# TalShor/SciLMM

Measured on AMD Instinct MI355X. Metric: REML factorize+solve nnz(L)/s (simulated pedigree, fp64), higher is better.
Workload: dtype f64

## Files before the change

### scilmm_amd/csrc/dev.h

```cpp
#pragma once
#include <hip/hip_runtime.h>

#include <algorithm>
#include <cstdlib>
#include <optional>
#include <string>
#include <type_traits>
#include <vector>

#include "../../include/scilmm_hip.h"
#include "plan_types.h"
#include "handles.h"

namespace scilmm {

struct Tuning {
  int reserve_cus = 0;
  int side_streams = 2;
  bool no_mfma = false;
  bool trsm_lite = true;
  std::optional<bool> dense;
  std::optional<bool> outside;
  bool outside_merge = true;
  std::optional<int> outside_chunks;
  bool outside_prio = false;
  std::optional<double> cell_limit;
  bool no_lookahead = false;
  int look_depth = 2;
  bool host_cells = false;
  bool no_splitk = false;
  int64_t target_items = 1024;
  int64_t min_item = 24;
  int64_t max_item = 96;
  std::optional<int64_t> dense_items;
  int64_t dense_fill = 256;
  std::optional<bool> dense_taper;
  std::optional<int> dist_group;
  bool dist_nosplit = false;
  int chain_cap = 2048;
  int chain_wide = 12;
  bool no_chain = false;
  int64_t push_slice = 512;
  bool shadow = true;
  int chain_wide_t = 256;
  int chain_full_t = 768;
  bool sinv_generic = false;
};

inline Tuning read_tuning() {
  Tuning t;
  const char* gate = getenv("SCILMM_TUNING");
  if (!(gate && gate[0] == '1')) return t;
  auto env = [](const char* name) { return getenv(name); };
  auto is1 = [&](const char* name) { const char* e = env(name); return e && e[0] == '1'; };
  auto not0 = [&](const char* name) { const char* e = env(name); return !(e && e[0] == '0'); };
  const char* e;
  if ((e = env("SCILMM_RESERVE_CUS"))) t.reserve_cus = atoi(e);
  if ((e = env("SCILMM_SIDE_STREAMS"))) t.side_streams = atoi(e);
  t.no_mfma = is1("SCILMM_NO_MFMA");
  t.trsm_lite = not0("SCILMM_TRSM_LITE");
  if ((e = env("SCILMM_DENSE"))) t.dense = e[0] != '0';
  if ((e = env("SCILMM_OUTSIDE"))) t.outside = e[0] != '0';
  t.outside_merge = not0("SCILMM_OUTSIDE_MERGE");
  if ((e = env("SCILMM_OUTSIDE_CHUNKS"))) t.outside_chunks = atoi(e);
  t.outside_prio = is1("SCILMM_OUTSIDE_PRIO");
  if ((e = env("SCILMM_CELL_LIMIT"))) t.cell_limit = atof(e);
  t.no_lookahead = is1("SCILMM_NO_LOOKAHEAD");
  if ((e = env("SCILMM_LOOK_DEPTH"))) t.look_depth = std::max(1, atoi(e));
  t.host_cells = is1("SCILMM_HOST_CELLS");
  t.no_splitk = is1("SCILMM_NO_SPLITK");
  if ((e = env("SCILMM_TARGET_ITEMS"))) t.target_items = atoll(e);
  if ((e = env("SCILMM_MIN_ITEM"))) t.min_item = atoll(e);
  if ((e = env("SCILMM_MAX_ITEM"))) t.max_item = atoll(e);
  if ((e = env("SCILMM_DENSE_ITEMS"))) t.dense_items = atoll(e);
  if ((e = env("SCILMM_DENSE_FILL"))) t.dense_fill = atoll(e);
  if ((e = env("SCILMM_DENSE_TAPER"))) t.dense_taper = e[0] == '1';
  if ((e = env("SCILMM_DIST_GROUP"))) t.dist_group = atoi(e);
  t.dist_nosplit = is1("SCILMM_DIST_NOSPLIT");
  if ((e = env("SCILMM_CHAIN_CAP"))) t.chain_cap = atoi(e);
  if ((e = env("SCILMM_CHAIN_WIDE"))) t.chain_wide = atoi(e);
  t.no_chain = is1("SCILMM_NO_CHAIN");
  if ((e = env("SCILMM_PUSH_SLICE"))) t.push_slice = atoll(e);
  t.shadow = not0("SCILMM_SHADOW");
  if ((e = env("SCILMM_CHAIN_WIDE_T"))) t.chain_wide_t = atoi(e);
  if ((e = env("SCILMM_CHAIN_FULL_T"))) t.chain_full_t = atoi(e);
  t.sinv_generic = is1("SCILMM_SINV_GENERIC");
  return t;
}

inline bool verbose() { return getenv("SCILMM_VERBOSE") != nullptr; }

struct Dev {
  int device = 0;
  hipStream_t stream = nullptr;
  Tuning tune;
  int prio_lo = 0, prio_hi = 0;
  DevSym v{};
  std::vector<void*> allocs;
  int32_t* d_level_tiles = nullptr;
  int32_t* d_level_fronts = nullptr;
  int32_t* d_level_pairs = nullptr;
  int32_t* d_all_fronts = nullptr;
  std::vector<double*> vals;
  std::vector<uint8_t> have_vals;
  double* W = nullptr;
  double* X = nullptr;
  double* IO = nullptr;
  size_t io_cap = 0;
  double* partial = nullptr;
  size_t partial_cap = 0;
  double* d_out = nullptr;
  bool use_mfma = true;
  bool trsm_lite = true;
  hipEvent_t ev[8];
  scilmm_timing timing{};
  bool quad_pending = false;
  bool attrs_set = false;
  ComboDesc* d_combos = nullptr;
  UpdWork* d_work = nullptr;
  std::vector<int64_t> work_ptr;
  UpdWork* d_work_early = nullptr;
  std::vector<int64_t> early_ptr;
  int64_t max_slots = 0;
  hipStream_t side = nullptr;
  hipStream_t side2 = nullptr;
  hipStream_t side3 = nullptr;
  int nside = 2;
  bool serial_early = false;
  std::vector<hipEvent_t> lev_ev;
  hipEvent_t ev_asm = nullptr;
  hipEvent_t ev_x0 = nullptr, ev_x1 = nullptr;
  int32_t* d_tile_pslot = nullptr;
  int32_t* d_tile_pnseg = nullptr;
  int32_t* d_tile_pslot_e = nullptr;
  int32_t* d_tile_pnseg_e = nullptr;
  int32_t* d_red_tiles_e = nullptr;
  std::vector<int64_t> red_ptr_e;
  std::vector<int64_t> lev_cost_e, lev_cost_l;
// ... 23 lines not shown
  std::vector<int32_t> lv_ptr, lv_fronts, lv_tiles, lv_pairs;
  std::vector<int64_t> lv_tile_ptr, lv_tile_mid, lv_pair_ptr;
  int32_t* d_lmul_tiles = nullptr;
  int64_t n_lmul_tiles = 0;
  DenseWork* d_dwork_b = nullptr;
  std::vector<int64_t> dbatch_ptr;
  std::vector<hipEvent_t> batch_ev;
  std::vector<hipEvent_t> bpev;
  std::vector<int32_t> last_own_level;
  hipStream_t bstream = nullptr;
  hipStream_t comm = nullptr;
  std::vector<hipEvent_t> done_ev;
  double* ACC = nullptr;
  int32_t* d_col_front = nullptr;
  int64_t* d_yoff = nullptr;
  double* d_ybuf = nullptr;
  int32_t* d_sinv_pre_tiles = nullptr;
  std::vector<int64_t> sinv_pre_ptr;
  std::vector<int32_t> sinv_tail_front;
  int32_t* d_sinv_tail_fronts = nullptr;
  SinvWork* d_sinv_work = nullptr;
  std::vector<int64_t> sinv_work_ptr;
  bool work_external = false;
  bool outside_on = false;
  int32_t tail_level = 0;
  std::vector<uint8_t> outside_desc;
  OutsideWork* d_owork = nullptr;
  int32_t* d_grp_next = nullptr;
  int32_t* d_grp_t0 = nullptr;
  int64_t n_owork = 0;
  int32_t* d_tail_front = nullptr;
  uint8_t* d_keep_front = nullptr;
  hipStream_t outside_st = nullptr;
  std::vector<int64_t> ochunk_ptr;
  std::vector<hipEvent_t> out_evs;
  std::vector<int32_t> out_wait_chunk;
  bool dense_on = false;
  int front_bits = 64;
  double* d_zeros = nullptr;
  DenseWork* d_dwork_e = nullptr;
  DenseWork* d_dwork_l = nullptr;
  std::vector<int64_t> dwork_e_ptr, dwork_l_ptr;
  std::vector<int64_t> dwork_l_mid;
  int64_t n_late_split = 0;
  int look_depth = 2;
  int rhs_pending = -1;
  int32_t chain_T = 0, chain_l0 = 0;
  int32_t* d_chain = nullptr;
  int32_t* d_colmap = nullptr;
  int32_t* d_cf_ptr = nullptr;
  ChainPair* d_cf = nullptr;
  int32_t* d_cb_ptr = nullptr;
  ChainPair* d_cb = nullptr;
  int64_t* d_cg_ptr = nullptr;
  int32_t* d_cg_pairs = nullptr;
  int64_t chain_groups = 0;
  int32_t* d_cg_slot = nullptr;
  int32_t* d_fold = nullptr;
  int64_t n_fold = 0;
  double* d_push_partial = nullptr;
  int32_t* d_chain_flags = nullptr;
  int32_t* d_chain_err = nullptr;
  int32_t* h_chain_err = nullptr;
  int32_t chain_epoch = 0;
  std::vector<hipEvent_t> pev;
  bool det = false;
  PullPlan pull{};
  int32_t* d_pull_level_segs = nullptr;
  int32_t* d_pull_fold = nullptr;
  double* d_pull_partial = nullptr;
  uint8_t* d_chain_mask = nullptr;
  const int64_t* d_pat_rowptr = nullptr;
  const int64_t* d_pat_rowslot = nullptr;
  const int32_t* d_pat_rowcol = nullptr;
  int64_t n_float_atomic = 0;
  double* scan_partial = nullptr;
  size_t scan_partial_cap = 0;
  double* gram_partial = nullptr;
  size_t gram_partial_cap = 0;
  const int32_t* d_iperm = nullptr;
  hipEvent_t scan_ev[4] = {nullptr, nullptr, nullptr, nullptr};
  bool scan_pending = false;
  double scan_ms[3] = {0.0, 0.0, 0.0};
  hipEvent_t gxe_ev[2] = {nullptr, nullptr};
  bool gxe_pending = false;
  double gxe_ms[2] = {0.0, 0.0};
};

#define HIPCHK(call)                                                                                   \
  do {                                                                                                 \
    hipError_t _e = (call);                                                                            \
    if (_e != hipSuccess) {                                                                            \
      sym->err = std::string(#call) + ": " + hipGetErrorString(_e);                                    \
      return SCILMM_ERR_DEVICE;                                                                        \
    }                                                                                                  \
  } while (0)

#define TRY(call)                      \
  do {                                 \
    int _rc = (call);                  \
    if (_rc != SCILMM_OK) return _rc;  \
  } while (0)

struct DevScratch {
  std::string* const err;
  std::vector<void*> held;
// ... 100 lines not shown
```

### scilmm_amd/csrc/kernels.hip.h

```cpp
#pragma once
#include <hip/hip_runtime.h>
#ifndef SCILMM_UPD_WAVES
#define SCILMM_UPD_WAVES 2
#endif
#include <stdint.h>

#include "plan_types.h"

namespace scilmm {

typedef double d4 __attribute__((ext_vector_type(4)));

constexpr int NJB = NB / 16;
constexpr int KCS = 16;
constexpr int LDA = TM + 16;
constexpr int LDB = NB + 16;
constexpr int LDP = 34;

__device__ __forceinline__ d4 mfma_f64(double a, double b, d4 c) {
  return __builtin_amdgcn_mfma_f64_16x16x4f64(a, b, c, 0, 0, 0);
}

__global__ void k_assemble(int64_t nnz, const int64_t* __restrict__ dst, ValPtrs vp, double* __restrict__ L) {
  int64_t stride = (int64_t)gridDim.x * blockDim.x;
  for (int64_t e = (int64_t)blockIdx.x * blockDim.x + threadIdx.x; e < nnz; e += stride) {
    double v = 0.0;
#pragma unroll
    for (int k = 0; k < 8; ++k)
      if (k < vp.count) v += vp.s2[k] * vp.v[k][e];
    const int64_t d = dst[e];
    if (d >= 0) L[d] = v;
  }
}

__global__ void k_add_rows(int64_t count, const double* __restrict__ src, double* __restrict__ dst) {
  const int64_t i = (int64_t)blockIdx.x * blockDim.x + threadIdx.x;
  if (i < count) dst[i] += src[i];
}

__global__ void k_status_pack(const int32_t* __restrict__ status, double* __restrict__ out) { *out = (double)*status; }
__global__ void k_status_unpack(const double* __restrict__ in, int32_t* __restrict__ status) { *status = (int32_t)*in; }

__global__ void k_add_diag(int32_t n, const int64_t* __restrict__ diag_dst, ValPtrs vp, double* __restrict__ L) {
  int32_t j = blockIdx.x * blockDim.x + threadIdx.x;
  if (j >= n) return;
  double v = 0.0;
#pragma unroll
  for (int k = 0; k < 8; ++k)
    if (k < vp.count) v += vp.s2[k] * vp.v[k][j];
  if (diag_dst[j] >= 0) L[diag_dst[j]] += v;
}

template <bool MFMA>
__device__ __forceinline__ void tile_mma(const double* __restrict__ As, const double* __restrict__ Bs, int kc4, int ncb,
                                         int lane, int wv, d4 (&acc)[NJB][2]) {
  const int li = lane & 15, lk = lane >> 4;
  if (MFMA) {
    const double* ap = As + lk * LDA + 32 * wv + li;
// ... 1785 lines not shown
}

template <int MODE>
__global__ __launch_bounds__(256) void k_pull_fold(DevSym S, const int32_t* __restrict__ fold, const double* __restrict__ partial,
                                                   double* __restrict__ W, int32_t rp) {
  const int32_t s = fold[3 * blockIdx.x], slot0 = fold[3 * blockIdx.x + 1], ns = fold[3 * blockIdx.x + 2];
  const int c_lo = blockIdx.y * CW;
  const int rpl = min(CW, rp - c_lo);
  const int32_t c0 = S.sn_start[s], w = S.sn_start[s + 1] - c0;
  const int cc = threadIdx.x % CW;
  if (cc >= rpl) return;
  for (int k = threadIdx.x / CW; k < w; k += 256 / CW) {
    double sum = 0.0;
    for (int sl = 0; sl < ns; ++sl) sum += partial[((int64_t)(slot0 + sl) * NB + k) * rp + c_lo + cc];
    if (MODE == 0) W[(int64_t)(c0 + k) * rp + c_lo + cc] -= sum;
    else W[(int64_t)(c0 + k) * rp + c_lo + cc] = sum;
  }
}


__device__ __forceinline__ bool chain_wait(const int32_t* flag, int32_t epoch, int32_t* err, int behind) {
  int spins = 0;
  int32_t seen = __hip_atomic_load(err + 1, __ATOMIC_RELAXED, __HIP_MEMORY_SCOPE_AGENT);
  unsigned long long t_seen = wall_clock64();
  while (__hip_atomic_load(flag, __ATOMIC_RELAXED, __HIP_MEMORY_SCOPE_AGENT) < epoch) {
    if (behind == 0) __builtin_amdgcn_s_sleep(1);
    else
      for (int z = 0; z < min(behind, 8); ++z) __builtin_amdgcn_s_sleep(127);
    if ((++spins & 255) == 0) {
      if (__hip_atomic_load(err, __ATOMIC_RELAXED, __HIP_MEMORY_SCOPE_AGENT) != 0) return false;
      const int32_t now = __hip_atomic_load(err + 1, __ATOMIC_RELAXED, __HIP_MEMORY_SCOPE_AGENT);
      const unsigned long long t = wall_clock64();
      if (now != seen) {
        seen = now;
        t_seen = t;
      } else if (t - t_seen > 100000000ull) {
        __hip_atomic_store(err, 1, __ATOMIC_RELAXED, __HIP_MEMORY_SCOPE_AGENT);
        return false;
      }
    }
  }
  return true;
}

#ifndef SCILMM_CHAIN_WAVES
#define SCILMM_CHAIN_WAVES 2
#endif
#ifdef SCILMM_CHAIN_PROF
__device__ unsigned long long g_chain_prof[8 * 4096];
#define CPROF(slot) do { if (c == 0 && tid == 0 && i < 4096 && !BWD) g_chain_prof[8 * i + (slot)] = wall_clock64(); } while (0)
#else
#define CPROF(slot) do {} while (0)
#endif
template <bool MFMA, bool BWD, int NCTW>
__global__ __launch_bounds__(512, NCTW == 2 ? SCILMM_CHAIN_WAVES : 1) void k_chain(DevSym S, int32_t T, const int32_t* __restrict__ chain,
                                               const int32_t* __restrict__ pair_ptr, const ChainPair* __restrict__ pairs,
                                               const int32_t* __restrict__ colmap, const double* __restrict__ L,
                                               const double* __restrict__ invD, const double* W, double* X, int32_t rp,
                                               int32_t ncw, int32_t* flags, int32_t epoch, int32_t* err, int32_t* ticket) {
  constexpr int CW = 16 * NCTW, LDW = NCTW == 2 ? 48 : NCTW == 4 ? 80 : 112, NCT = NCTW;
  static_assert(NCTW == 2 || NCTW == 4 || NCTW == 7, "k_chain: 32-, 64- or 112-column windows");
  __shared__ __attribute__((aligned(16))) double Ys[NB * LDW];
  __shared__ int s_ok, s_ready, s_ticket;
  const int tid = threadIdx.x, lane = tid & 63, wv = tid >> 6;
  const int li = lane & 15, lk = lane >> 4;
  if (tid == 0) s_ticket = atomicAdd(ticket, 1);
  __syncthreads();
  const int32_t lin = s_ticket;
  const int32_t ord = lin / ncw, c = lin - ord * ncw;
  const int32_t i = BWD ? T - 1 - ord : ord;
  const int c_lo = c * CW;
  const int rpl = min(CW, rp - c_lo);
  const int ncn = rpl >> 4;
  const int32_t s = chain[i];
  const int32_t c0 = S.sn_start[s], w = S.sn_start[s + 1] - c0;
  const int32_t m = (int32_t)(S.sn_rowptr[s + 1] - S.sn_rowptr[s]);
  const double* I = invD + S.inv_off[s];
  constexpr int NK = NB / 4;
  const int jrow = 16 * wv + li;
  const int32_t e0 = pair_ptr[i], e1 = pair_ptr[i + 1];
  if (wv == 0) {
    int ready = 0;
    bool open = true;
    for (int32_t base = e0; base < e1 && open; base += 64) {
      bool r = false;
      if (base + lane < e1)
        r = __hip_atomic_load(flags + (int64_t)pairs[base + lane].other * ncw + c, __ATOMIC_RELAXED, __HIP_MEMORY_SCOPE_AGENT) >= epoch;
      const unsigned long long b = __ballot(r);
      const int lead = (~b == 0ull) ? 64 : __builtin_ctzll(~b);
      ready += lead;
      open = lead == 64;
    }
    if (lane == 0) s_ready = ready;
  }
  const int w4 = (w + 3) & ~3;
  const int kbeg = BWD ? 16 * wv : 0;
  const int kend = BWD ? w4 : min(w4, 16 * (wv + 1));
  double iv[NK];
  auto load_iv = [&]() {
    const int jc = jrow < w ? jrow : 0;
    const uint32_t voff = (uint32_t)(BWD ? jc * w + lk : lk * w + jc);
    const int klast = uniform_int(max(w4 - 4, 0)), wu = uniform_int(w);
    const double* Ib = invD + uniform_i64(S.inv_off[s]);
#pragma unroll
    for (int u = 0; u < NK; ++u) {
      const int ku = min(4 * u, klast);
      iv[u] = ld_off(Ib + (BWD ? ku : ku * wu), voff * 8u);
    }
  };
  const double* Yin = BWD ? (const double*)X : W;
  double yv[NCT][4];
  auto load_yv = [&]() {
#pragma unroll
    for (int cn = 0; cn < NCT; ++cn)
#pragma unroll
      for (int r = 0; r < 4; ++r) {
        const int jr = 16 * wv + lk + 4 * r;
        yv[cn][r] = (jr < w && cn < ncn) ? Yin[(int64_t)(c0 + jr) * rp + c_lo + 16 * cn + li] : 0.0;
      }
  };
  if (NCTW == 2) load_yv();
  d4 acc[NCT];
#pragma unroll
  for (int cn = 0; cn < NCT; ++cn) acc[cn] = (d4){0.0, 0.0, 0.0, 0.0};
  __syncthreads();
  const int32_t nready = s_ready;
  bool ok = true;
  auto load_frag = [&](int32_t e, double (&av)[NK]) {
    const ChainPair pr = pairs[e];
    if (!BWD) {
      const int32_t so = chain[pr.other];
      const int32_t wo = S.sn_start[so + 1] - S.sn_start[so];
      const int64_t md = S.sn_rowptr[so + 1] - S.sn_rowptr[so];
      int q = jrow - pr.jp0;
      if (pr.jp0 < 0) q = colmap[pr.map + jrow];
      const bool rowok = q >= 0 && q < pr.nq;
      const double* Pj = L + uniform_i64(S.sn_loff[so] + pr.p0);
      const int64_t mdu = uniform_int((int)md);
      const uint32_t voff = (uint32_t)(lk * (int)md + (rowok ? q : 0));
      const int klast = uniform_int(max(((wo + 3) & ~3) - 4, 0));
#pragma unroll
      for (int u = 0; u < NK; ++u) av[u] = ld_off(Pj + (int64_t)min(4 * u, klast) * mdu, voff * 8u);
    } else {
      const double* Pi = L + uniform_i64(S.sn_loff[s] + pr.p0);
      const uint32_t voff = (uint32_t)((jrow < w ? jrow : 0) * m + lk);
      const int klast = uniform_int(max(((pr.nq + 3) & ~3) - 4, 0));
#pragma unroll
      for (int u = 0; u < NK; ++u) av[u] = ld_off(Pi + min(4 * u, klast), voff * 8u);
    }
  };
  auto consume = [&](int32_t e, double (&av)[NK]) {
    const ChainPair pr = pairs[e];
    const int32_t so = chain[pr.other];
    const int32_t co = S.sn_start[so], wo = S.sn_start[so + 1] - co;
    const int kn = BWD ? ((pr.nq + 3) & ~3) : ((wo + 3) & ~3);
    bool rowok;
    if (!BWD) {
      int q = jrow - pr.jp0;
      if (pr.jp0 < 0) q = colmap[pr.map + jrow];
      rowok = q >= 0 && q < pr.nq;
    } else {
      rowok = jrow < w;
    }
    const int kvalid = BWD ? pr.nq : wo;
    if (NCTW == 2 && e == e1 - 1) load_iv();
    if (e - e0 >= nready) {
      if (tid == 0) s_ok = chain_wait(flags + (int64_t)pr.other * ncw + c, epoch, err, e1 - 1 - e) ? 1 : 0;
      if (e == e1 - 1) CPROF(0);
      __syncthreads();
      ok = s_ok != 0;
    }
    if (ok) {
      const int nx = BWD ? pr.nq : wo;
#pragma unroll
      for (int cbase = 0; cbase < LDW; cbase += 64) {
        const int cc = cbase + (tid & 63);
        if (cc < LDW) {
          double xv[NB / 8];
#pragma unroll
// ... 1 lines not shown
            const int k = (tid >> 6) + 8 * u;
            xv[u] = 0.0;
            if (k < nx && cc < rpl) {
              int64_t xr;
              if (!BWD) xr = co + k;
              else xr = (pr.jp0 >= 0) ? co + pr.jp0 + k : S.sn_rows[S.sn_rowptr[s] + pr.p0 + k];
              xv[u] = X[xr * rp + c_lo + cc];
            }
          }
#pragma unroll
          for (int u = 0; u < NB / 8; ++u) {
            const int k = (tid >> 6) + 8 * u;
            if (k < kn) Ys[k * LDW + cc] = xv[u];
          }
        }
      }
    }
    __syncthreads();
    if (e == e1 - 1) CPROF(1);
    if (ok) {
      if (MFMA) {
#pragma unroll
        for (int u = 0; u < NK; ++u)
          if (4 * u < kn) {
#pragma unroll
            for (int cn = 0; cn < NCT; ++cn)
              if (cn < ncn)
                acc[cn] = mfma_f64((rowok && 4 * u + lk < kvalid) ? av[u] : 0.0, Ys[(4 * u + lk) * LDW + 16 * cn + li], acc[cn]);
          }
      } else {
        for (int k = 0; k < kn; ++k) {
#pragma unroll
          for (int r = 0; r < 4; ++r) {
            const int jr = 16 * wv + lk + 4 * r;
            double a = 0.0;
            if (!BWD) {
              const int64_t md = S.sn_rowptr[so + 1] - S.sn_rowptr[so];
              int q = jr - pr.jp0;
              if (pr.jp0 < 0) q = colmap[pr.map + jr];
              if (q >= 0 && q < pr.nq && k < wo) a = L[S.sn_loff[so] + (int64_t)k * md + pr.p0 + q];
            } else {
              if (jr < w && k < pr.nq) a = L[S.sn_loff[s] + (int64_t)jr * m + pr.p0 + k];
            }
#pragma unroll
            for (int cn = 0; cn < NCT; ++cn)
              if (cn < ncn) acc[cn][r] += a * Ys[k * LDW + 16 * cn + li];
          }
        }
      }
    }
    __syncthreads();
    if (e == e1 - 1) CPROF(2);
  };
  if (NCTW == 2 && e0 == e1) load_iv();
  for (int32_t e = e0; e < e1 && ok; ++e) {
    double av[NK];
    load_frag(e, av);
    consume(e, av);
  }
  if (NCTW != 2) {
    load_iv();
    load_yv();
  }
  if (ok) {
#pragma unroll
    for (int cn = 0; cn < NCT; ++cn)
#pragma unroll
      for (int r = 0; r < 4; ++r) {
        const int jr = 16 * wv + lk + 4 * r;
        if (jr < w4) Ys[jr * LDW + 16 * cn + li] = (jr < w && cn < ncn) ? yv[cn][r] - acc[cn][r] : 0.0;
      }
  }
  __syncthreads();
  CPROF(3);
  if (ok && 16 * wv < w) {
    d4 xa[NCT];
#pragma unroll
    for (int cn = 0; cn < NCT; ++cn) xa[cn] = (d4){0.0, 0.0, 0.0, 0.0};
    if (MFMA) {
#pragma unroll
      for (int u = 0; u < NK; ++u)
        if (4 * u >= kbeg && 4 * u < kend) {
#pragma unroll
          for (int cn = 0; cn < NCT; ++cn)
            if (cn < ncn)
              xa[cn] = mfma_f64((jrow < w && 4 * u + lk < w) ? iv[u] : 0.0, Ys[(4 * u + lk) * LDW + 16 * cn + li], xa[cn]);
        }
    } else {
      for (int k = kbeg; k < kend && k < w; ++k)
#pragma unroll
        for (int r = 0; r < 4; ++r) {
          const int jr = 16 * wv + lk + 4 * r;
          const double a = (jr < w) ? (BWD ? I[(int64_t)jr * w + k] : I[(int64_t)k * w + jr]) : 0.0;
#pragma unroll
          for (int cn = 0; cn < NCT; ++cn)
            if (cn < ncn) xa[cn][r] += a * Ys[k * LDW + 16 * cn + li];
        }
    }
#pragma unroll
    for (int cn = 0; cn < NCT; ++cn)
      if (cn < ncn)
#pragma unroll
        for (int r = 0; r < 4; ++r) {
          const int jr = 16 * wv + lk + 4 * r;
          if (jr < w)
            __hip_atomic_store(&X[(int64_t)(c0 + jr) * rp + c_lo + 16 * cn + li], xa[cn][r], __ATOMIC_RELAXED, __HIP_MEMORY_SCOPE_AGENT);
        }
  }
  CPROF(4);
  __asm__ volatile("s_waitcnt vmcnt(0)" ::: "memory");
  __syncthreads();
  CPROF(5);
  if (tid == 0 && ok) {
    __hip_atomic_store(flags + (int64_t)i * ncw + c, epoch, __ATOMIC_RELAXED, __HIP_MEMORY_SCOPE_AGENT);
    __hip_atomic_fetch_add(err + 1, 1, __ATOMIC_RELAXED, __HIP_MEMORY_SCOPE_AGENT);
  }
}

__global__ __launch_bounds__(256) void k_quad(DevSym S, int64_t nnz, int64_t slots_per_wave,
                                              const double* __restrict__ vals, const double* __restrict__ U,
                                              int32_t rp, double* __restrict__ partial) {
  const int lane = threadIdx.x & 63;
  const int64_t wave = (int64_t)blockIdx.x * 4 + (threadIdx.x >> 6);
  const int64_t e0 = wave * slots_per_wave;
  const int64_t e1 = min(nnz, e0 + slots_per_wave);
  double t0 = 0.0, t1 = 0.0;
  if (e0 < e1) {
    int32_t lo = 0, hi = S.n;
    while (lo < hi) {
      int32_t mid = (lo + hi) >> 1;
      if (S.pat_colptr[mid + 1] <= e0) lo = mid + 1; else hi = mid;
    }
// ... 673 lines not shown
```

### scilmm_amd/csrc/plan.hip

```cpp
#include <hip/hip_runtime.h>

#include <algorithm>
#include <atomic>
#include <chrono>
#include <functional>
#include <thread>
#include <cmath>
#include <cstdio>
#include <cstdlib>
#include <cstring>
#include <string>
#include <vector>

#include "dev.h"
#include "cellplan.hip.h"
#include "host_threads.h"

namespace scilmm {

void dev_free(void* p) {
  Dev* D = (Dev*)p;
  if (!D) return;
  for (void* a : D->allocs) (void)hipFree(a);
  for (double* v : D->vals)
// ... 1457 lines not shown
      for (size_t g = 0; g + 1 < gptr.size(); ++g) {
        int64_t rows = 0;
        for (int64_t q = gptr[g]; q < gptr[g + 1]; ++q) rows += gpairs[3 * q + 2] - gpairs[3 * q + 1];
        const int64_t nsl = (rows + slice_rows - 1) / slice_rows;
        if (nsl <= 1) {
          gptr2.push_back((int64_t)gp2.size() / 3);
          gp2.insert(gp2.end(), gpairs.begin() + 3 * gptr[g], gpairs.begin() + 3 * gptr[g + 1]);
          gslot.push_back(-1);
          continue;
        }
        const int64_t per = (rows + nsl - 1) / nsl;
        fold.push_back(gpairs[3 * gptr[g]]);
        fold.push_back(nslots);
        int32_t made = 0;
        int64_t acc = 0;
        gptr2.push_back((int64_t)gp2.size() / 3);
        gslot.push_back(nslots + made);
        ++made;
        for (int64_t q = gptr[g]; q < gptr[g + 1]; ++q) {
          int32_t a = gpairs[3 * q + 1];
          const int32_t b = gpairs[3 * q + 2];
          while (a < b) {
            if (acc == per) {
              gptr2.push_back((int64_t)gp2.size() / 3);
              gslot.push_back(nslots + made);
              ++made;
              acc = 0;
            }
            const int32_t take = (int32_t)std::min<int64_t>(b - a, per - acc);
            gp2.push_back(gpairs[3 * q]);
            gp2.push_back(a);
            gp2.push_back(a + take);
            a += take;
            acc += take;
          }
        }
        fold.push_back(made);
        nslots += made;
      }
      gptr2.push_back((int64_t)gp2.size() / 3);
      gptr.swap(gptr2);
      gpairs.swap(gp2);
      D->n_fold = (int64_t)fold.size() / 3;
      if (nslots > 0) {
        void* pp = nullptr;
        HIPCHK(hipMalloc(&pp, sizeof(double) * (size_t)nslots * NB * RPMAX));
        D->allocs.push_back(pp);
        D->d_push_partial = (double*)pp;
      }
      if (fold.empty()) fold.assign(3, 0);
      if (gslot.empty()) gslot.push_back(-1);
    }
    D->chain_groups = (int64_t)gptr.size() - 1;
    if (fl.empty()) fl.push_back(ChainPair{0, 0, 0, 0, 0});
    if (bl.empty()) bl.push_back(ChainPair{0, 0, 0, 0, 0});
    if (colmap.empty()) colmap.push_back(-1);
    if ((st = upload(sym, D, colmap, &D->d_colmap)) != SCILMM_OK) return st;
    if (gpairs.empty()) gpairs.assign(3, 0);
    const int64_t n_ranges = (int64_t)gpairs.size() / 3;
    if ((st = upload(sym, D, chain, &D->d_chain)) != SCILMM_OK) return st;
    if ((st = upload(sym, D, fptr, &D->d_cf_ptr)) != SCILMM_OK) return st;
    if ((st = upload(sym, D, bptr, &D->d_cb_ptr)) != SCILMM_OK) return st;
    if ((st = upload(sym, D, fl, &D->d_cf)) != SCILMM_OK) return st;
    if ((st = upload(sym, D, bl, &D->d_cb)) != SCILMM_OK) return st;
    if ((st = upload(sym, D, gptr, &D->d_cg_ptr)) != SCILMM_OK) return st;
    if ((st = upload(sym, D, gpairs, &D->d_cg_pairs)) != SCILMM_OK) return st;
    if ((st = upload(sym, D, gslot, &D->d_cg_slot)) != SCILMM_OK) return st;
    if ((st = upload(sym, D, fold, &D->d_fold)) != SCILMM_OK) return st;
    std::vector<int32_t> zeros((size_t)T * (RPMAX / CW) + 4, 0);
    if ((st = upload(sym, D, zeros, &D->d_chain_flags)) != SCILMM_OK) return st;
    D->d_chain_err = D->d_chain_flags + (size_t)T * (RPMAX / CW);
    HIPCHK(hipHostMalloc((void**)&D->h_chain_err, sizeof(int32_t), hipHostMallocDefault));
    *D->h_chain_err = 0;
    if (pb.verbose)
      fprintf(stderr, "[scilmm plan] chain sweep: %d fronts (levels %d..%d), %lld inner pairs (%lld column maps), %lld outside pairs in %lld groups\n",
              T, l0, S.nlevels - 1, (long long)fl.size(), (long long)(colmap.size() / NB), (long long)outside.size(), (long long)D->chain_groups);
    (void)n_ranges;
  }
  return SCILMM_OK;
}

}

int ensure_device(scilmm_symbolic* sym, Dev** out) {
  if (sym->device) {
    *out = (Dev*)sym->device;
    return SCILMM_OK;
  }
  int ndev = 0;
  if (hipGetDeviceCount(&ndev) != hipSuccess || ndev == 0) {
    sym->err = "no HIP device available (the numeric phase has no CPU fallback)";
    return SCILMM_ERR_DEVICE;
  }
  PlanBuild pb;
  pb.verbose = verbose();
  {
    const hipError_t stale = hipGetLastError();
    if (stale != hipSuccess && pb.verbose)
      fprintf(stderr, "[scilmm plan] cleared a stale HIP error of this thread: %s\n", hipGetErrorString(stale));
  }
  Dev* D = new Dev();
  sym->device = D;
  sym->device_free = dev_free;
  if (hipGetDevice(&D->device) != hipSuccess) D->device = 0;
  for (auto& e : D->ev) e = nullptr;
  D->tune = read_tuning();
  D->det = sym->deterministic;
  D->use_mfma = !D->tune.no_mfma;
  D->trsm_lite = D->tune.trsm_lite;
#ifdef SCILMM_DIAG
  const char* ab = getenv("SCILMM_ABLATE");
  D->ablate = ab ? atoi(ab) : 0;
#endif
  int st;
  if ((st = create_streams_and_events(sym, D)) != SCILMM_OK) return st;
  if ((st = check_block_widths(sym)) != SCILMM_OK) return st;
  if ((st = plan_ownership(sym, D, pb)) != SCILMM_OK) return st;
  if ((st = choose_tail_paths(sym, D)) != SCILMM_OK) return st;
  if (D->outside_on && (st = plan_outside(sym, D, pb)) != SCILMM_OK) return st;
  if (!sym->S->combos_built) {
    scilmm::build_tile_combos(sym->S, D->world > 1 ? D->keep_front.data() : nullptr, D->dense_on,
                              D->outside_on ? D->outside_desc.data() : nullptr);
    pb.lap("tile combos");
  } else {
    D->dense_on = false;
  }
  if ((st = upload_symbolic(sym, D)) != SCILMM_OK) return st;
  pb.lap("symbolic arrays -> device");
  if (D->det) {
// ... 89 lines not shown
```

### scilmm_amd/csrc/plan_types.h

```cpp
#pragma once
#include <stdint.h>
#ifndef SCILMM_KC
#define SCILMM_KC 16
#endif
#ifndef SCILMM_NB
#define SCILMM_NB 128
#endif
#ifndef SCILMM_CW
#define SCILMM_CW 32
#endif

namespace scilmm {

constexpr int NB = SCILMM_NB;
constexpr int TM = 128;
constexpr int KC = SCILMM_KC;
constexpr int RPMAX = 128;
constexpr int CW = SCILMM_CW;

struct DevSym {
  int32_t n, nsuper;
  const int32_t* sn_start;
  const int64_t* sn_rowptr;
  const int32_t* sn_rows;
// ... 16 lines not shown
  double s2[8];
  int32_t count;
};

struct ComboDesc {
  int64_t loff;
  int64_t rowoff;
  int32_t md, wd;
  int32_t ta, nt;
  int32_t p0, nq;
  int32_t ip0;
  int32_t jp0;
  int32_t ilo, ihi;
  int32_t jlo, jhi;
};

struct UpdWork {
  int32_t tile;
  int32_t slot;
  int64_t cb, ce;
};

struct DenseWork {
  int32_t front;
  int32_t ti0;
  int32_t ntiles;
  int32_t k0, k1;
  int32_t slot0, slot1;
  int32_t pad;
};

struct OutsideWork {
  int32_t d;
  int32_t t0;
  int32_t bi, bj;
};

struct CellSrc { int64_t st, sq; int32_t md, wd; };

struct PullPlan {
  const int32_t* seg_front;
  const int64_t* seg_ptr;
  const int32_t* seg_slot;
  const int32_t* front_seg;
};

struct ChainPair {
  int32_t other;
  int32_t p0, nq;
  int32_t jp0;
  int32_t map;
};

struct SinvOwner {
  int64_t loff;
  const int32_t* rows;
  int32_t c0, m;
  int32_t tail;
};

struct SinvWork {
  int32_t front;
  int32_t q;
  int32_t ka, kb;
};

}
```

### scilmm_amd/csrc/sweep.hip.h

```cpp
#pragma once

namespace {

int ensure_work(scilmm_symbolic* sym, Dev* D) {
  const Symbolic& S = *sym->S;
  size_t bytes = (size_t)std::max(S.n, 1) * RPMAX * sizeof(double);
  if (D->world > 1 && !D->work_external) {
    sym->err = "multi-GPU: scilmm_dist_set_work has not been called (the sweeps' buffers must be addressable by the communication layer)";
    return SCILMM_ERR_STATE;
  }
  if (!D->W) HIPCHK(hipMalloc((void**)&D->W, bytes));
  if (!D->X) HIPCHK(hipMalloc((void**)&D->X, bytes));
  return set_attrs(sym, D);
}

inline int rp_of(int rc) { return (rc + 15) & ~15; }

struct Sweep : SweepLaunch {
  scilmm_symbolic* const sym;
  const Symbolic& S;
  int64_t tot = 0;
  int chain_wide_T = 0, chain_full_T = 0;
  bool mid_recorded = false;

  Sweep(scilmm_factor* f, Dev* d) : SweepLaunch{d, f, d->stream}, sym(f->sym), S(*f->sym->S) {}

  void set_block(int rc) {
    rp = rp_of(rc);
    gy = (unsigned)((rp + CW - 1) / CW);
    tot = (int64_t)S.n * rp;
    const Tuning tune = read_tuning();
    chain_wide_T = tune.chain_wide_t;
    chain_full_T = tune.chain_full_t;
  }

  int mark_mid() {
    if (!mid_recorded) HIPCHK(hipEventRecord(D->ev[4], st));
    mid_recorded = true;
    return SCILMM_OK;
  }

  int chain(bool bwd) {
    const bool mf = D->use_mfma;
    const bool wide = D->chain_T >= chain_wide_T;
    const bool full = D->chain_T >= chain_full_T && rp > 64;
    const int32_t cwc = full ? 112 : wide ? 64 : 32;
    const int32_t gyc = (int32_t)((rp + cwc - 1) / cwc);
    const unsigned grid = (unsigned)D->chain_T * (unsigned)gyc;
    const int32_t ep = ++D->chain_epoch;
    HIPCHK(hipMemsetAsync(D->d_chain_err + 2, 0, sizeof(int32_t), st));
    const int32_t* cptr = bwd ? (const int32_t*)D->d_cb_ptr : (const int32_t*)D->d_cf_ptr;
    const ChainPair* cpairs = bwd ? (const ChainPair*)D->d_cb : (const ChainPair*)D->d_cf;
#define SCILMM_CHAIN_LAUNCH(MF, BW, NC)                                                                                                  \
  hipLaunchKernelGGL((k_chain<MF, BW, NC>), dim3(grid), dim3(512), 0, st, D->v, D->chain_T, (const int32_t*)D->d_chain, cptr, cpairs, \
                     (const int32_t*)D->d_colmap, (const double*)fac->L, (const double*)fac->invD, (const double*)D->W, D->X, rp, gyc,  \
                     D->d_chain_flags, ep, D->d_chain_err, D->d_chain_err + 2)
    if (mf) {
      if (bwd) { if (full) SCILMM_CHAIN_LAUNCH(true, true, 7); else if (wide) SCILMM_CHAIN_LAUNCH(true, true, 4); else SCILMM_CHAIN_LAUNCH(true, true, 2); }
      else { if (full) SCILMM_CHAIN_LAUNCH(true, false, 7); else if (wide) SCILMM_CHAIN_LAUNCH(true, false, 4); else SCILMM_CHAIN_LAUNCH(true, false, 2); }
    } else {
      if (bwd) SCILMM_CHAIN_LAUNCH(false, true, 2); else SCILMM_CHAIN_LAUNCH(false, false, 2);
    }
#undef SCILMM_CHAIN_LAUNCH
    return SCILMM_OK;
  }

  void pull(int32_t la, int32_t lb, bool lmul, const uint8_t* skip) {
    const int64_t g0 = S.pull_level_ptr[(size_t)la], g1 = S.pull_level_ptr[(size_t)lb];
    const int64_t h0 = S.pull_fold_ptr[(size_t)la], h1 = S.pull_fold_ptr[(size_t)lb];
    double* out = lmul ? D->X : D->W;
    fwd_pull(lmul, D->d_pull_level_segs + g0, g1 - g0, skip, lmul ? D->W : D->X, out);
    pull_fold(lmul, D->d_pull_fold + 3 * h0, h1 - h0, out);
  }
  void pull_groups(int32_t lo, bool lmul, const uint8_t* skip) {
    for (size_t q = 0; q + 1 < S.pull_group_ptr.size(); ++q) {
      const int32_t la = std::max(lo, S.pull_group_ptr[q]), lb = S.pull_group_ptr[q + 1];
      if (la < lb) pull(la, lb, lmul, skip);
    }
  }

  int32_t level_end() const { return D->chain_T > 0 ? D->chain_l0 : S.nlevels; }

  int forward_single() {
    const int32_t lend = level_end();
    for (int32_t l = 0; l < lend; ++l) {
      const int64_t t0 = S.level_tile_ptr[l], t1 = S.level_tile_ptr[l + 1];
      const int32_t f0 = S.level_ptr[l], f1 = S.level_ptr[l + 1];
      if (f1 == f0) continue;
      if (D->det && l > 0) pull(l, l + 1, false, nullptr);
      diag_solve(false, D->d_level_fronts + f0, f1 - f0, D->W, D->X);
      if (!D->det) fwd(0, (f1 - f0) > 1, D->d_level_tiles + t0, t1 - t0, D->X, D->W);
    }
    if (D->chain_T > 0) {
      if (D->det) pull_groups(lend, false, D->d_chain_mask);
      TRY(chain(false));
    }
    return SCILMM_OK;
  }

  int backward_single() {
    const int32_t lend = level_end();
    if (D->chain_T > 0) {
      TRY(chain(true));
      bwd_push(D->d_cg_pairs, D->chain_groups, D->d_cg_ptr, D->d_cg_slot, D->d_push_partial);
      if (D->chain_groups > 0 && D->n_fold > 0)
        hipLaunchKernelGGL(k_push_fold, dim3((unsigned)D->n_fold, gy), dim3(256), 0, st, D->v, (const int32_t*)D->d_fold,
                           (const double*)D->d_push_partial, D->X, rp);
    }
    for (int32_t l = lend - 1; l >= 0; --l) {
      diag_solve(true, D->d_level_fronts + S.level_ptr[l], S.level_ptr[l + 1] - S.level_ptr[l], D->X, D->X);
      bwd_push(D->d_level_pairs + S.level_pair_ptr[l], S.level_pair_ptr[l + 1] - S.level_pair_ptr[l]);
    }
    return SCILMM_OK;
  }
// ... 167 lines not shown
```

Before: 1.419 billion.

## Pipeline chain-sweep pair loop with precomputed descriptors and register prefetch

Adds a pipelined variant of the chain solve kernel for the 64-column window. It runs over precomputed 32-byte per-pair descriptors built at plan time, double-buffers the L fragments and X loads across pairs, and scans readiness in runs so dependent pairs can stream without per-pair waits. It also splits the full-width diagonal multiply across waves, and lowers the threshold for using the wide kernel so more chains take this path. The cost is extra device memory for the descriptors, more kernel variants and register pressure, and a more complex synchronisation scheme.

```diff
diff --git a/scilmm_amd/csrc/dev.h b/scilmm_amd/csrc/dev.h
--- a/scilmm_amd/csrc/dev.h
+++ b/scilmm_amd/csrc/dev.h
@@ -42,8 +42,10 @@
   bool no_chain = false;
   int64_t push_slice = 512;
   bool shadow = true;
-  int chain_wide_t = 256;
+  int chain_wide_t = 160;
   int chain_full_t = 768;
+  bool chain_pipe = true;
+  int chain_stagger = 0;
   bool sinv_generic = false;
 };
 
@@ -84,6 +86,8 @@
   t.shadow = not0("SCILMM_SHADOW");
   if ((e = env("SCILMM_CHAIN_WIDE_T"))) t.chain_wide_t = atoi(e);
   if ((e = env("SCILMM_CHAIN_FULL_T"))) t.chain_full_t = atoi(e);
+  t.chain_pipe = not0("SCILMM_CHAIN_PIPE");
+  if ((e = env("SCILMM_CHAIN_STAGGER"))) t.chain_stagger = std::max(0, atoi(e));
   t.sinv_generic = is1("SCILMM_SINV_GENERIC");
   return t;
 }
@@ -213,6 +217,9 @@
   ChainPair* d_cf = nullptr;
   int32_t* d_cb_ptr = nullptr;
   ChainPair* d_cb = nullptr;
+  ChainDesc* d_cfd = nullptr;
+  ChainDesc* d_cbd = nullptr;
+  int64_t chain_desc_bytes = 0;
   int64_t* d_cg_ptr = nullptr;
   int32_t* d_cg_pairs = nullptr;
   int64_t chain_groups = 0;
diff --git a/scilmm_amd/csrc/kernels.hip.h b/scilmm_amd/csrc/kernels.hip.h
--- a/scilmm_amd/csrc/kernels.hip.h
+++ b/scilmm_amd/csrc/kernels.hip.h
@@ -4,6 +4,7 @@
 #define SCILMM_UPD_WAVES 2
 #endif
 #include <stdint.h>
+#include <type_traits>
 
 #include "plan_types.h"
 
@@ -1895,16 +1896,19 @@
 #else
 #define CPROF(slot) do {} while (0)
 #endif
-template <bool MFMA, bool BWD, int NCTW>
+template <bool MFMA, bool BWD, int NCTW, bool PIPE>
 __global__ __launch_bounds__(512, NCTW == 2 ? SCILMM_CHAIN_WAVES : 1) void k_chain(DevSym S, int32_t T, const int32_t* __restrict__ chain,
                                                const int32_t* __restrict__ pair_ptr, const ChainPair* __restrict__ pairs,
+                                               const ChainDesc* __restrict__ descs,
                                                const int32_t* __restrict__ colmap, const double* __restrict__ L,
                                                const double* __restrict__ invD, const double* W, double* X, int32_t rp,
-                                               int32_t ncw, int32_t* flags, int32_t epoch, int32_t* err, int32_t* ticket) {
+                                               int32_t ncw, int32_t* flags, int32_t epoch, int32_t* err, int32_t* ticket,
+                                               int32_t stagger) {
+  static_assert(MFMA || !PIPE, "k_chain: the scalar form has no pipelined loop");
   constexpr int CW = 16 * NCTW, LDW = NCTW == 2 ? 48 : NCTW == 4 ? 80 : 112, NCT = NCTW;
   static_assert(NCTW == 2 || NCTW == 4 || NCTW == 7, "k_chain: 32-, 64- or 112-column windows");
   __shared__ __attribute__((aligned(16))) double Ys[NB * LDW];
-  __shared__ int s_ok, s_ready, s_ticket;
+  __shared__ int s_ok, s_ready, s_deep, s_ticket;
   const int tid = threadIdx.x, lane = tid & 63, wv = tid >> 6;
   const int li = lane & 15, lk = lane >> 4;
   if (tid == 0) s_ticket = atomicAdd(ticket, 1);
@@ -1922,7 +1926,7 @@
   constexpr int NK = NB / 4;
   const int jrow = 16 * wv + li;
   const int32_t e0 = pair_ptr[i], e1 = pair_ptr[i + 1];
-  if (wv == 0) {
+  if (!PIPE && wv == 0) {
     int ready = 0;
     bool open = true;
     for (int32_t base = e0; base < e1 && open; base += 64) {
@@ -1967,7 +1971,7 @@
 #pragma unroll
   for (int cn = 0; cn < NCT; ++cn) acc[cn] = (d4){0.0, 0.0, 0.0, 0.0};
   __syncthreads();
-  const int32_t nready = s_ready;
+  const int32_t nready = PIPE ? 0 : s_ready;
   bool ok = true;
   auto load_frag = [&](int32_t e, double (&av)[NK]) {
     const ChainPair pr = pairs[e];
@@ -2075,13 +2079,217 @@
     __syncthreads();
     if (e == e1 - 1) CPROF(2);
   };
+  constexpr bool HOP_EARLY = PIPE && NCTW == 4;
   if (NCTW == 2 && e0 == e1) load_iv();
-  for (int32_t e = e0; e < e1 && ok; ++e) {
-    double av[NK];
-    load_frag(e, av);
-    consume(e, av);
-  }
-  if (NCTW != 2) {
+  if constexpr (!PIPE) {
+    for (int32_t e = e0; e < e1 && ok; ++e) {
+      double av[NK];
+      load_frag(e, av);
+      consume(e, av);
+    }
+  } else if (e0 < e1) {
+    constexpr bool PF_FRAG = NCTW != 7;
+    const int32_t e1u = uniform_int(e1);
+    int32_t e = uniform_int(e0);
+    int32_t fin = e;
+    auto ldesc = [&](int32_t q) __attribute__((always_inline)) { return descs[min(q, e1u - 1)]; };
+    constexpr int XL = NCTW == 2 ? 32 : 64, XR = 512 / XL, XU = NB / XR, XP = (CW + XL - 1) / XL;
+    const int xc = tid & (XL - 1), xk = tid / XL;
+    const int64_t rowbase = BWD ? S.sn_rowptr[s] : 0;
+    double xv[XP][XU];
+    auto opaque = [](int v) __attribute__((always_inline)) {
+      __asm__ volatile("" : "+v"(v));
+      return v;
+    };
+    auto xload = [&](int32_t xrow, int32_t nx, int32_t jp0, int32_t map) __attribute__((always_inline)) {
+      if (BWD && jp0 < 0) {
+        const int32_t* rows = S.sn_rows + (rowbase + map);
+#pragma unroll
+        for (int p = 0; p < XP; ++p)
+#pragma unroll
+          for (int u = 0; u < XU; ++u) {
+            const int kc = max(min(xk + XR * u, nx - 1), 0), cc = XL * p + xc;
+            xv[p][u] = X[(int64_t)rows[kc] * rp + c_lo + (cc < rpl ? cc : 0)];
+          }
+      } else {
+        const double* Xb = X + uniform_i64((int64_t)xrow * rp + c_lo);
+#pragma unroll
+        for (int p = 0; p < XP; ++p)
+#pragma unroll
+          for (int u = 0; u < XU; ++u) {
+            const int kc = max(min(xk + XR * u, nx - 1), 0), cc = XL * p + xc;
+            xv[p][u] = ld_off(Xb, (uint32_t)(kc * rp + (cc < rpl ? cc : 0)) * 8u);
+          }
+      }
+    };
+    auto xwrite = [&](int32_t nx) __attribute__((always_inline)) {
+      const int kn = (nx + 3) & ~3;
+      double* Yw = Ys + opaque(xk * LDW + xc);
+#pragma unroll
+      for (int p = 0; p < XP; ++p)
+#pragma unroll
+        for (int u = 0; u < XU; ++u) {
+          const int k = xk + XR * u, cc = XL * p + xc;
+          if (cc < CW && k < kn) Yw[XR * u * LDW + XL * p] = (k < nx && cc < rpl) ? xv[p][u] : 0.0;
+        }
+    };
+    auto frag = [&](const ChainDesc& d, int32_t qm, double (&av)[NK], bool& rowok) __attribute__((always_inline)) {
+      const int klast = max(((d.depth + 3) & ~3) - 4, 0);
+      const double* P = L + d.loff;
+      if (!BWD) {
+        const int q = d.jp0 < 0 ? qm : jrow - d.jp0;
+        rowok = q >= 0 && q < d.nq;
+        const uint32_t voff = (uint32_t)(lk * d.ld + (rowok ? q : 0));
+#pragma unroll
+        for (int u = 0; u < NK; ++u) av[u] = ld_off(P + (int64_t)min(4 * u, klast) * d.ld, voff * 8u);
+      } else {
+        rowok = jrow < w;
+        const uint32_t voff = (uint32_t)((rowok ? jrow : 0) * d.ld + lk);
+#pragma unroll
+        for (int u = 0; u < NK; ++u) av[u] = ld_off(P + min(4 * u, klast), voff * 8u);
+      }
+    };
+    auto cmap = [&](const ChainDesc& d) __attribute__((always_inline)) { return BWD ? 0 : colmap[d.map + jrow]; };
+    const int ncnu = uniform_int(ncn);
+    auto mult = [&](const ChainDesc& d, double (&av)[NK], bool rowok) __attribute__((always_inline)) {
+      const int kn = (d.depth + 3) & ~3, kvalid = d.depth;
+      const double* Yb = Ys + opaque(lk * LDW + li);
+      if (kvalid == NB && ncnu == NCT) {
+#pragma unroll
+        for (int u = 0; u < NK; ++u)
+#pragma unroll
+          for (int cn = 0; cn < NCT; ++cn) acc[cn] = mfma_f64(rowok ? av[u] : 0.0, Yb[4 * u * LDW + 16 * cn], acc[cn]);
+      } else {
+        const int lko = opaque(lk);
+#pragma unroll
+        for (int u = 0; u < NK; ++u)
+          if (4 * u < kn) {
+#pragma unroll
+            for (int cn = 0; cn < NCT; ++cn)
+              if (cn < ncnu) acc[cn] = mfma_f64((rowok && 4 * u + lko < kvalid) ? av[u] : 0.0, Yb[4 * u * LDW + 16 * cn], acc[cn]);
+          }
+      }
+    };
+    if (stagger > 0 && e1u - e > stagger) {
+      if (tid == 0) s_ok = chain_wait(flags + (int64_t)ldesc(e1u - 1 - stagger).other * ncw + c, epoch, err, stagger) ? 1 : 0;
+      __syncthreads();
+      ok = uniform_int(s_ok) != 0;
+    }
+    ChainDesc d0 = ldesc(e), d1 = ldesc(e + 1), d2 = ldesc(e + 2), d3;
+    double avA[NK], avB[NK];
+    bool rokA, rokB = false;
+    int32_t qm1 = cmap(d1), qm2;
+    frag(d0, cmap(d0), avA, rokA);
+    auto run_step = [&](double (&cur)[NK], bool& rokc, double (&nxt)[NK], bool& rokn, bool more) __attribute__((always_inline)) {
+      d3 = ldesc(e + 3);
+      qm2 = cmap(d2);
+      if (PF_FRAG) frag(d1, qm1, nxt, rokn);
+      __builtin_amdgcn_sched_barrier(0);
+      xwrite(d0.depth);
+      __syncthreads();
+      xload(more ? d1.xrow : d0.xrow, more ? d1.depth : d0.depth, more ? d1.jp0 : d0.jp0, more ? d1.map : d0.map);
+      __builtin_amdgcn_sched_barrier(0);
+      {
+        const double* Yb = Ys + opaque(lk * LDW + li);
+#pragma unroll
+        for (int u = 0; u < NK; ++u)
+#pragma unroll
+          for (int cn = 0; cn < NCT; ++cn) acc[cn] = mfma_f64(rokc ? cur[u] : 0.0, Yb[4 * u * LDW + 16 * cn], acc[cn]);
+      }
+      if (!PF_FRAG) {
+        __builtin_amdgcn_sched_barrier(0);
+        frag(d1, qm1, cur, rokc);
+      }
+      __syncthreads();
+      d0 = d1, d1 = d2, d2 = d3, qm1 = qm2;
+      ++e;
+    };
+    auto single = [&](bool last) __attribute__((always_inline)) {
+      if (!last) {
+        d3 = ldesc(e + 3);
+        qm2 = cmap(d2);
+        if (PF_FRAG) frag(d1, qm1, avB, rokB);
+      } else {
+        if (NCTW == 2 || HOP_EARLY) load_iv();
+        if (HOP_EARLY) load_yv();
+      }
+      if (e >= fin) {
+        if (tid == 0) s_ok = chain_wait(flags + (int64_t)d0.other * ncw + c, epoch, err, e1u - 1 - e) ? 1 : 0;
+        __syncthreads();
+        ok = uniform_int(s_ok) != 0;
+      }
+      if (last) CPROF(0);
+      if (ok) {
+        xload(d0.xrow, d0.depth, d0.jp0, d0.map);
+        xwrite(d0.depth);
+      }
+      __syncthreads();
+      if (last) CPROF(1);
+      if (ok) mult(d0, avA, rokA);
+      if (!last && !PF_FRAG) {
+        __builtin_amdgcn_sched_barrier(0);
+        frag(d1, qm1, avA, rokA);
+      }
+      __syncthreads();
+      if (last) CPROF(2);
+      if (!last) {
+        if (PF_FRAG) {
+#pragma unroll
+          for (int u = 0; u < NK; ++u) avA[u] = avB[u];
+          rokA = rokB;
+        }
+        d0 = d1, d1 = d2, d2 = d3, qm1 = qm2;
+      }
+      ++e;
+    };
+    int32_t runfin = e;
+    while (e < e1u - 1 && ok) {
+      if (e >= runfin) {
+        if (wv == 0) {
+          int ready = 0, deep = 0;
+          bool open = true, opend = true;
+          for (int32_t base = e; base < e1u && open; base += 64) {
+            bool r = false, d = false;
+            if (base + lane < e1u) {
+              r = __hip_atomic_load(flags + (int64_t)descs[base + lane].other * ncw + c, __ATOMIC_RELAXED, __HIP_MEMORY_SCOPE_AGENT) >= epoch;
+              d = r && descs[base + lane].depth == NB;
+            }
+            const unsigned long long b = __ballot(r), bd = __ballot(d);
+            const int lead = (~b == 0ull) ? 64 : __builtin_ctzll(~b);
+            const int leadd = (~bd == 0ull) ? 64 : __builtin_ctzll(~bd);
+            ready += lead;
+            if (opend) deep += leadd;
+            open = lead == 64;
+            opend = opend && leadd == 64;
+          }
+          if (lane == 0) s_ready = ready, s_deep = deep;
+        }
+        __syncthreads();
+        fin = e + uniform_int(s_ready);
+        runfin = e + uniform_int(s_deep);
+      }
+      const int32_t run_end = e + ((min(runfin, e1u - 1) - e) & ~1);
+      if (e < run_end) {
+        xload(d0.xrow, d0.depth, d0.jp0, d0.map);
+        while (e < run_end) {
+          if (PF_FRAG) {
+            run_step(avA, rokA, avB, rokB, true);
+            run_step(avB, rokB, avA, rokA, e + 1 < run_end);
+          } else {
+            run_step(avA, rokA, avA, rokA, true);
+            run_step(avA, rokA, avA, rokA, e + 1 < run_end);
+          }
+        }
+      } else {
+        single(false);
+      }
+    }
+    if (ok) single(true);
+  } else if (HOP_EARLY) {
+    load_iv();
+    load_yv();
+  }
+  if (NCTW != 2 && !HOP_EARLY) {
     load_iv();
     load_yv();
   }
@@ -2100,7 +2308,26 @@
     d4 xa[NCT];
 #pragma unroll
     for (int cn = 0; cn < NCT; ++cn) xa[cn] = (d4){0.0, 0.0, 0.0, 0.0};
-    if (MFMA) {
+    if (MFMA && w == NB && uniform_int(ncn) == NCT) {
+      const double* Yd = Ys + lk * LDW + li;
+      auto diag_wave = [&](auto WV) __attribute__((always_inline)) {
+        constexpr int u0 = BWD ? 4 * decltype(WV)::value : 0, u1 = BWD ? NK : 4 * (decltype(WV)::value + 1);
+#pragma unroll
+        for (int u = u0; u < u1; ++u)
+#pragma unroll
+          for (int cn = 0; cn < NCT; ++cn) xa[cn] = mfma_f64(iv[u], Yd[4 * u * LDW + 16 * cn], xa[cn]);
+      };
+      switch (uniform_int(wv)) {
+        case 0: diag_wave(std::integral_constant<int, 0>{}); break;
+        case 1: diag_wave(std::integral_constant<int, 1>{}); break;
+        case 2: diag_wave(std::integral_constant<int, 2>{}); break;
+        case 3: diag_wave(std::integral_constant<int, 3>{}); break;
+        case 4: diag_wave(std::integral_constant<int, 4>{}); break;
+        case 5: diag_wave(std::integral_constant<int, 5>{}); break;
+        case 6: diag_wave(std::integral_constant<int, 6>{}); break;
+        default: diag_wave(std::integral_constant<int, 7>{}); break;
+      }
+    } else if (MFMA) {
 #pragma unroll
       for (int u = 0; u < NK; ++u)
         if (4 * u >= kbeg && 4 * u < kend) {
diff --git a/scilmm_amd/csrc/plan.hip b/scilmm_amd/csrc/plan.hip
--- a/scilmm_amd/csrc/plan.hip
+++ b/scilmm_amd/csrc/plan.hip
@@ -1533,9 +1533,31 @@
       if (gslot.empty()) gslot.push_back(-1);
     }
     D->chain_groups = (int64_t)gptr.size() - 1;
+    std::vector<ChainDesc> fd(fl.size()), bd(bl.size());
+    for (int32_t i = 0; i < T; ++i) {
+      const int32_t s = chain[i];
+      const int32_t ms = (int32_t)(S.sn_rowptr[s + 1] - S.sn_rowptr[s]);
+      for (int32_t e = fptr[i]; e < fptr[i + 1]; ++e) {
+        const ChainPair& p = fl[(size_t)e];
+        const int32_t so = chain[p.other];
+        fd[(size_t)e] = ChainDesc{S.sn_loff[so] + p.p0, (int32_t)(S.sn_rowptr[so + 1] - S.sn_rowptr[so]), S.sn_start[so + 1] - S.sn_start[so],
+                                  S.sn_start[so], p.other, p.map, (int16_t)p.jp0, (int16_t)p.nq};
+      }
+      for (int32_t e = bptr[i]; e < bptr[i + 1]; ++e) {
+        const ChainPair& p = bl[(size_t)e];
+        const int32_t so = chain[p.other];
+        bd[(size_t)e] = ChainDesc{S.sn_loff[s] + p.p0, ms, p.nq, S.sn_start[so] + std::max(p.jp0, 0), p.other, p.p0, (int16_t)p.jp0, (int16_t)p.nq};
+      }
+    }
+    D->chain_desc_bytes = (int64_t)(fd.size() + bd.size()) * (int64_t)sizeof(ChainDesc);
     if (fl.empty()) fl.push_back(ChainPair{0, 0, 0, 0, 0});
     if (bl.empty()) bl.push_back(ChainPair{0, 0, 0, 0, 0});
-    if (colmap.empty()) colmap.push_back(-1);
+    if (fd.empty()) fd.push_back(ChainDesc{0, 0, 0, 0, 0, 0, 0, 0});
+    if (bd.empty()) bd.push_back(ChainDesc{0, 0, 0, 0, 0, 0, 0, 0});
+    const long long n_colmaps = (long long)(colmap.size() / NB);
+    colmap.resize(std::max(colmap.size(), (size_t)NB), -1);
+    if ((st = upload(sym, D, fd, &D->d_cfd)) != SCILMM_OK) return st;
+    if ((st = upload(sym, D, bd, &D->d_cbd)) != SCILMM_OK) return st;
     if ((st = upload(sym, D, colmap, &D->d_colmap)) != SCILMM_OK) return st;
     if (gpairs.empty()) gpairs.assign(3, 0);
     const int64_t n_ranges = (int64_t)gpairs.size() / 3;
@@ -1554,8 +1576,8 @@
     HIPCHK(hipHostMalloc((void**)&D->h_chain_err, sizeof(int32_t), hipHostMallocDefault));
     *D->h_chain_err = 0;
     if (pb.verbose)
-      fprintf(stderr, "[scilmm plan] chain sweep: %d fronts (levels %d..%d), %lld inner pairs (%lld column maps), %lld outside pairs in %lld groups\n",
-              T, l0, S.nlevels - 1, (long long)fl.size(), (long long)(colmap.size() / NB), (long long)outside.size(), (long long)D->chain_groups);
+      fprintf(stderr, "[scilmm plan] chain sweep: %d fronts (levels %d..%d), %lld inner pairs (%lld column maps, %lld descriptor bytes), %lld outside pairs in %lld groups\n",
+              T, l0, S.nlevels - 1, (long long)fl.size(), n_colmaps, (long long)D->chain_desc_bytes, (long long)outside.size(), (long long)D->chain_groups);
     (void)n_ranges;
   }
   return SCILMM_OK;
diff --git a/scilmm_amd/csrc/plan_types.h b/scilmm_amd/csrc/plan_types.h
--- a/scilmm_amd/csrc/plan_types.h
+++ b/scilmm_amd/csrc/plan_types.h
@@ -92,6 +92,17 @@
   int32_t map;
 };
 
+struct alignas(32) ChainDesc {
+  int64_t loff;
+  int32_t ld;
+  int32_t depth;
+  int32_t xrow;
+  int32_t other;
+  int32_t map;
+  int16_t jp0, nq;
+};
+static_assert(sizeof(ChainDesc) == 32, "ChainDesc: one 32-byte record per pair");
+
 struct SinvOwner {
   int64_t loff;
   const int32_t* rows;
diff --git a/scilmm_amd/csrc/sweep.hip.h b/scilmm_amd/csrc/sweep.hip.h
--- a/scilmm_amd/csrc/sweep.hip.h
+++ b/scilmm_amd/csrc/sweep.hip.h
@@ -20,7 +20,8 @@
   scilmm_symbolic* const sym;
   const Symbolic& S;
   int64_t tot = 0;
-  int chain_wide_T = 0, chain_full_T = 0;
+  int chain_wide_T = 0, chain_full_T = 0, chain_stagger = 0;
+  bool chain_pipe = true;
   bool mid_recorded = false;
 
   Sweep(scilmm_factor* f, Dev* d) : SweepLaunch{d, f, d->stream}, sym(f->sym), S(*f->sym->S) {}
@@ -32,6 +33,8 @@
     const Tuning tune = read_tuning();
     chain_wide_T = tune.chain_wide_t;
     chain_full_T = tune.chain_full_t;
+    chain_pipe = tune.chain_pipe;
+    chain_stagger = tune.chain_stagger;
   }
 
   int mark_mid() {
@@ -51,15 +54,26 @@
     HIPCHK(hipMemsetAsync(D->d_chain_err + 2, 0, sizeof(int32_t), st));
     const int32_t* cptr = bwd ? (const int32_t*)D->d_cb_ptr : (const int32_t*)D->d_cf_ptr;
     const ChainPair* cpairs = bwd ? (const ChainPair*)D->d_cb : (const ChainPair*)D->d_cf;
-#define SCILMM_CHAIN_LAUNCH(MF, BW, NC)                                                                                                  \
-  hipLaunchKernelGGL((k_chain<MF, BW, NC>), dim3(grid), dim3(512), 0, st, D->v, D->chain_T, (const int32_t*)D->d_chain, cptr, cpairs, \
-                     (const int32_t*)D->d_colmap, (const double*)fac->L, (const double*)fac->invD, (const double*)D->W, D->X, rp, gyc,  \
-                     D->d_chain_flags, ep, D->d_chain_err, D->d_chain_err + 2)
+    const ChainDesc* cdesc = bwd ? (const ChainDesc*)D->d_cbd : (const ChainDesc*)D->d_cfd;
+#define SCILMM_CHAIN_LAUNCH(MF, BW, NC, PP)                                                                                                  \
+  hipLaunchKernelGGL((k_chain<MF, BW, NC, PP>), dim3(grid), dim3(512), 0, st, D->v, D->chain_T, (const int32_t*)D->d_chain, cptr, cpairs,   \
+                     cdesc, (const int32_t*)D->d_colmap, (const double*)fac->L, (const double*)fac->invD, (const double*)D->W, D->X, rp, gyc, \
+                     D->d_chain_flags, ep, D->d_chain_err, D->d_chain_err + 2, (int32_t)chain_stagger)
+    const bool pipe = chain_pipe && wide && !full;
     if (mf) {
-      if (bwd) { if (full) SCILMM_CHAIN_LAUNCH(true, true, 7); else if (wide) SCILMM_CHAIN_LAUNCH(true, true, 4); else SCILMM_CHAIN_LAUNCH(true, true, 2); }
-      else { if (full) SCILMM_CHAIN_LAUNCH(true, false, 7); else if (wide) SCILMM_CHAIN_LAUNCH(true, false, 4); else SCILMM_CHAIN_LAUNCH(true, false, 2); }
+      if (bwd) {
+        if (full) SCILMM_CHAIN_LAUNCH(true, true, 7, false);
+        else if (pipe) SCILMM_CHAIN_LAUNCH(true, true, 4, true);
+        else if (wide) SCILMM_CHAIN_LAUNCH(true, true, 4, false);
+        else SCILMM_CHAIN_LAUNCH(true, true, 2, false);
+      } else {
+        if (full) SCILMM_CHAIN_LAUNCH(true, false, 7, false);
+        else if (pipe) SCILMM_CHAIN_LAUNCH(true, false, 4, true);
+        else if (wide) SCILMM_CHAIN_LAUNCH(true, false, 4, false);
+        else SCILMM_CHAIN_LAUNCH(true, false, 2, false);
+      }
     } else {
-      if (bwd) SCILMM_CHAIN_LAUNCH(false, true, 2); else SCILMM_CHAIN_LAUNCH(false, false, 2);
+      if (bwd) SCILMM_CHAIN_LAUNCH(false, true, 2, false); else SCILMM_CHAIN_LAUNCH(false, false, 2, false);
     }
 #undef SCILMM_CHAIN_LAUNCH
     return SCILMM_OK;
```

New measurement: 1.436 billion (median of 6 runs). +1.2%, better.
